# zeahmed/NeuralASR

Hardware: AMD Instinct MI355X
Metric: audio-frames/sec (fwd+bwd+CTC+Adam) at batch 16 per GPU (higher is better)
Workload: dtype f32

## Files before the change

neuralasr_amd/build.py:

```python
import os
import subprocess
import sys
from concurrent.futures import ThreadPoolExecutor

HERE = os.path.dirname(os.path.abspath(__file__))
CSRC = os.path.join(HERE, 'csrc')
LIB = os.path.join(HERE, 'libnasr.so')
KT_LIB = os.path.join(HERE, 'libnasr_kt.so')
KT_SRC = os.path.join(HERE, '..', 'tests', 'kernel_harness', 'harness.hip')
KT_OBJS = ['gemm.o', 'gemm_tph.o', 'optim.o']
SOURCES = ['gemm.hip', 'gemm_tph.hip', 'lstm.hip', 'lstm_persist.hip', 'lstm_wide.hip', 'ctc.hip', 'dense.hip', 'optim.hip', 'nasr_layout.hip',
           'nasr_rec.hip', 'nasr_batch.hip', 'nasr_pass.hip', 'nasr_api.hip', 'nasr_comm.hip', 'beam.cpp',
           'wavenet.hip', 'nasr_wavenet.hip', 'las.hip', 'las_beam.hip', 'nasr_las.hip', 'mfcc.hip', 'resample.hip']
HEADERS = [os.path.join(CSRC, 'kernels.h'), os.path.join(CSRC, 'lstm_device.h'), os.path.join(CSRC, 'nasr_ctx.h'), os.path.join(CSRC, 'wavenet.h'), os.path.join(CSRC, 'las.h'), os.path.join(CSRC, 'las_beam.h'), os.path.join(CSRC, 'resample.h'),
           os.path.join(HERE, '..', 'include', 'nasr.h')]
FLAGS = ['--offload-arch=gfx950', '-O3', '-std=c++17', '-fPIC', '-Wall', '-Wno-unused-function']


def _hipcc():
    for c in (os.environ.get('HIPCC'), '/opt/rocm/bin/hipcc', 'hipcc'):
        if c and (os.path.isabs(c) and os.path.exists(c) or not os.path.isabs(c)):
            return c
    return 'hipcc'


def _stale(target, deps):
    if not os.path.exists(target):
        return True
    t = os.path.getmtime(target)
    return any(os.path.getmtime(d) > t for d in deps if os.path.exists(d))


def build(force=False, verbose=False):
    hipcc = _hipcc()
    bdir = os.path.join(HERE, 'build')
    os.makedirs(bdir, exist_ok=True)
    jobs = []
    objs = []
    for s in SOURCES:
        src = os.path.join(CSRC, s)
        obj = os.path.join(bdir, os.path.splitext(s)[0] + '.o')
        objs.append(obj)
        if force or _stale(obj, [src] + HEADERS):
            jobs.append([hipcc] + FLAGS + ['-c', src, '-o', obj])

    def run(cmd):
        if verbose:
# ... 24 lines not shown
```

neuralasr_amd/csrc/gemm.hip:

```cpp
#include "kernels.h"

namespace nasr {

typedef float f32x16 __attribute__((ext_vector_type(16)));

constexpr int BM = 128, BN = 128, BK = 16, LDT = 132;

struct GemmParams {
  const float* A;
  const float* B;
  float* C;
  int M, N, K, lda, ldb, ldc;
  const int* a_map;
  int a_shift, a_rows;
  const int* c_map;
  const float* bias;
  int split_k, kchunk;
  float* slabs;
};

__device__ __forceinline__ int phys_row(const int* map, int shift, int rows, int logical) {
  int r = map ? map[logical] : logical + shift;
  return (r >= 0 && r < rows) ? r : -1;
}

__device__ __forceinline__ float4 ld4(const float* __restrict__ p) { return *reinterpret_cast<const float4*>(p); }
__device__ __forceinline__ float4 sel4(bool ok, float4 v) {
  return make_float4(ok ? v.x : 0.f, ok ? v.y : 0.f, ok ? v.z : 0.f, ok ? v.w : 0.f);
}

template <bool ACOL, bool BCOL>
__global__ __launch_bounds__(256, 2) void gemm_kernel(GemmParams p) {
  __shared__ __attribute__((aligned(16))) float As[2][BK][LDT];
  __shared__ __attribute__((aligned(16))) float Bs[2][BK][LDT];
  const int tid = threadIdx.x, lane = tid & 63, w = tid >> 6;
  const int m0 = blockIdx.y * BM, n0 = blockIdx.x * BN;
  const int kbeg = blockIdx.z * p.kchunk;
  const int kend = min(p.K, kbeg + p.kchunk);
  const int nk = (kend - kbeg + BK - 1) / BK;
  const float* __restrict__ Ag = p.A;
  const float* __restrict__ Bg = p.B;

  constexpr int NS = BK / 8, KQ = BK / 4;
  bool aok[NS], bok[NS];
  size_t ao[NS], bo[NS];
#pragma unroll
  for (int j = 0; j < NS; ++j) {
    const int idx = tid + 256 * j;
    const int r = idx / KQ, kq = idx % KQ, q = idx & 31;
    if (!ACOL) {
      const int pa = (m0 + r < p.M) ? phys_row(p.a_map, p.a_shift, p.a_rows, m0 + r) : -1;
// ... 78 lines not shown
        nb0 = Bs[buf][k][wn + li]; nb1 = Bs[buf][k][wn + 32 + li];
      }
      acc00 = __builtin_amdgcn_mfma_f32_32x32x2f32(a0, b0, acc00, 0, 0, 0);
      acc01 = __builtin_amdgcn_mfma_f32_32x32x2f32(a0, b1, acc01, 0, 0, 0);
      acc10 = __builtin_amdgcn_mfma_f32_32x32x2f32(a1, b0, acc10, 0, 0, 0);
      acc11 = __builtin_amdgcn_mfma_f32_32x32x2f32(a1, b1, acc11, 0, 0, 0);
      a0 = na0; a1 = na1; b0 = nb0; b1 = nb1;
    }
    if (more) NASR_LSTORE(buf ^ 1);
    __syncthreads();
  }
#undef NASR_GLOAD
#undef NASR_LSTORE

#pragma unroll
  for (int t = 0; t < 4; ++t) {
    const int mi = t >> 1, ni = t & 1;
    const f32x16 acc = t == 0 ? acc00 : t == 1 ? acc01 : t == 2 ? acc10 : acc11;
    const int col = n0 + wn + 32 * ni + li;
    if (col >= p.N) continue;
    const float bv = (p.bias && p.split_k == 1) ? p.bias[col] : 0.f;
#pragma unroll
    for (int r = 0; r < 16; ++r) {
      const int row = m0 + wm + 32 * mi + (r & 3) + 8 * (r >> 2) + 4 * lk;
      if (row >= p.M) continue;
      if (p.split_k > 1) {
        p.slabs[((size_t)blockIdx.z * p.M + row) * p.N + col] = acc[r];
      } else {
        const int pr = p.c_map ? p.c_map[row] : row;
        if (pr >= 0) p.C[(size_t)pr * p.ldc + col] = acc[r] + bv;
      }
    }
  }
}

__global__ __launch_bounds__(256) void gemm_reduce_kernel(GemmParams p) {
  const int64_t n4 = (int64_t)p.M * p.N / 4;
  for (int64_t i = blockIdx.x * (int64_t)blockDim.x + threadIdx.x; i < n4; i += (int64_t)gridDim.x * blockDim.x) {
    const int64_t e = i * 4;
    const int row = (int)(e / p.N), col = (int)(e % p.N);
    float4 s = *reinterpret_cast<const float4*>(p.slabs + e);
    for (int k = 1; k < p.split_k; ++k) {
      const float4 v = *reinterpret_cast<const float4*>(p.slabs + (size_t)k * p.M * p.N + e);
      s.x += v.x; s.y += v.y; s.z += v.z; s.w += v.w;
    }
    if (p.bias) { s.x += p.bias[col]; s.y += p.bias[col + 1]; s.z += p.bias[col + 2]; s.w += p.bias[col + 3]; }
    const int pr = p.c_map ? p.c_map[row] : row;
    if (pr >= 0) *reinterpret_cast<float4*>(p.C + (size_t)pr * p.ldc + col) = s;
  }
}

int gemm_pick_split(int M, int N, int K) {
  const int tiles = ((M + BM - 1) / BM) * ((N + BN - 1) / BN);
  int s = (512 + tiles - 1) / tiles;
  const int max_s = K / 128;
  if (s > max_s) s = max_s;
  if (s < 1) s = 1;
  return s;
}

void launch_gemm(const GemmDesc& g, hipStream_t st) {
  GemmParams p;
  p.A = g.A; p.B = g.B; p.C = g.C;
  p.M = g.M; p.N = g.N; p.K = g.K; p.lda = g.lda; p.ldb = g.ldb; p.ldc = g.ldc;
  p.a_map = g.a_map; p.a_shift = g.a_shift; p.a_rows = g.a_rows; p.c_map = g.c_map; p.bias = g.bias;
  p.split_k = g.split_k < 1 ? 1 : g.split_k;
  p.slabs = g.slabs;
  int kt = (g.K + BK - 1) / BK;
  int per = (kt + p.split_k - 1) / p.split_k;
  p.kchunk = per * BK;
  p.split_k = (kt + per - 1) / per;
  dim3 grid((g.N + BN - 1) / BN, (g.M + BM - 1) / BM, p.split_k), block(256);
  if (!g.a_col && !g.b_col) hipLaunchKernelGGL((gemm_kernel<false, false>), grid, block, 0, st, p);
  else if (g.a_col && !g.b_col) hipLaunchKernelGGL((gemm_kernel<true, false>), grid, block, 0, st, p);
  else if (!g.a_col && g.b_col) hipLaunchKernelGGL((gemm_kernel<false, true>), grid, block, 0, st, p);
  else hipLaunchKernelGGL((gemm_kernel<true, true>), grid, block, 0, st, p);
  if (p.split_k > 1) {
    int64_t n4 = (int64_t)g.M * g.N / 4;
    int blocks = (int)((n4 + 255) / 256);
    if (blocks > 2048) blocks = 2048;
    hipLaunchKernelGGL(gemm_reduce_kernel, dim3(blocks), dim3(256), 0, st, p);
  }
}

}
```

neuralasr_amd/csrc/gemm_tph.hip:

```cpp
#include "kernels.h"

#include <cstdlib>

namespace nasr {

namespace {

typedef _Float16 f16x8 __attribute__((ext_vector_type(8)));
typedef float f32x16 __attribute__((ext_vector_type(16)));
typedef __attribute__((address_space(3))) void* lds_ptr_t;
typedef const __attribute__((address_space(1))) void* gbl_ptr_t;

constexpr int HTB = 1024;
constexpr int TPH_LDS = 2 * 64 * HTB;

__device__ __attribute__((aligned(1024))) unsigned char g_tph_zero[HTB];

__device__ __forceinline__ int tph_slot(int r, int h) { return ((r << 1) | (h ^ ((r >> 3) & 1))) << 4; }

struct GemmTPHParams {
  const unsigned char* A;
  const unsigned char* B;
  float* C;
  int M, N;
  int nkbA, nkbB;
  int kbs;
  int ldc;
  int a_kb_shift;
  const float* bias;
  const float* a_inv;
  const float* b_inv;
  int split_k, kb_chunk;
  float* slabs;
  int nbatch;
  long long a_bstride, b_bstride, c_bstride, ainv_bstride, binv_bstride;
  int a_kb_shift1;
  int swz, gx, gy, gz, pr, pc, pz, sr, sc, sz;
  const int* c_map;
};

__device__ __forceinline__ void emit_h2(const float (&x)[8], float s, unsigned char* dst) {
  f16x8 p1, p2;
#pragma unroll
  for (int e = 0; e < 8; ++e) {
    const float v = x[e] * s;
    const _Float16 h1 = (_Float16)v;
    p1[e] = h1;
    p2[e] = (_Float16)(v - (float)h1);
  }
  *reinterpret_cast<f16x8*>(dst) = p1;
  *reinterpret_cast<f16x8*>(dst + HTB) = p2;
}

}

__global__ __launch_bounds__(256) void absmax_part_kernel(const float* __restrict__ src, int rows, int K, int ld,
                                                          float* __restrict__ rowpart, float* __restrict__ colpart) {
  __shared__ float rm[64][5], cm[4][64];
  const int t = threadIdx.x;
  const int r0 = blockIdx.y * 64, c0 = blockIdx.x * 64;
  const int cq = t & 15, rq = t >> 4;
  float cmax[4] = {0.f, 0.f, 0.f, 0.f};
#pragma unroll
  for (int i = 0; i < 4; ++i) {
    const int r = rq + 16 * i;
    float4 v = make_float4(0.f, 0.f, 0.f, 0.f);
// ... 360 lines not shown
#pragma unroll
        for (int j = 0; j < 2; ++j) acc[i][j] = chain3(acc[i][j], a[i], b[j]);
    }
  }

  const int li = lane & 31, lh = lane >> 5;
  const float* ainv = p.a_inv + (bz ? p.ainv_bstride : 0);
  const float* binv = p.b_inv + (bz ? p.binv_bstride : 0);
#pragma unroll
  for (int mi = 0; mi < TMW; ++mi)
#pragma unroll
    for (int ni = 0; ni < 2; ++ni) {
      const int col = n0 + wn * 64 + 32 * ni + li;
      if (col >= p.N) continue;
      const float bv = (p.bias && p.split_k == 1) ? p.bias[col] : 0.f;
      const float sb = binv[col];
#pragma unroll
      for (int r = 0; r < 16; ++r) {
        const int row = m0 + wm * (32 * TMW) + 32 * mi + (r & 3) + 8 * (r >> 2) + 4 * lh;
        if (row >= p.M) continue;
        const float v = acc[mi][ni][r] * (ainv[row] * sb);
        if (p.split_k > 1) {
          p.slabs[((size_t)bzz * p.M + row) * p.N + col] = v;
        } else {
          if constexpr (CMAP) {
            const int orow = p.c_map[row];
            if (orow >= 0) p.C[(size_t)bz * p.c_bstride + (size_t)orow * p.ldc + col] = v + bv;
          } else {
            p.C[(size_t)bz * p.c_bstride + (size_t)row * p.ldc + col] = v + bv;
          }
        }
      }
    }
}

constexpr int TPH_LDS_SIDE = 2 * 40 * HTB;

hipError_t gemm_tph_prepare() {
  hipError_t e = hipFuncSetAttribute(reinterpret_cast<const void*>(&gemm_tph_kernel<4, 2, 4>),
                                     hipFuncAttributeMaxDynamicSharedMemorySize, TPH_LDS);
  for (const void* f : {reinterpret_cast<const void*>(&gemm_tph_kernel<3, 2, 4>), reinterpret_cast<const void*>(&gemm_tph_kernel<4, 2, 4, true>),
                        reinterpret_cast<const void*>(&gemm_tph_kernel<3, 2, 4, true>)})
    if (e == hipSuccess) e = hipFuncSetAttribute(f, hipFuncAttributeMaxDynamicSharedMemorySize, TPH_LDS);
  if (e == hipSuccess)
    e = hipFuncSetAttribute(reinterpret_cast<const void*>(&gemm_tph_kernel<4, 1, 3>), hipFuncAttributeMaxDynamicSharedMemorySize,
                            TPH_LDS_SIDE);
  return e;
}

int gemm_tph_pick_split(int M, int N, int K, int nbatch) {
  const int tm = gemm_tp_tile_rows(M), tn = 256;
  const int tiles = ((M + tm - 1) / tm) * ((N + tn - 1) / tn) * (nbatch > 1 ? 2 : 1);
  const int kbs = (K + 15) / 16;
  const double kstep = 1.3e-6 * tm / 256.0;
  const double slab = (double)(nbatch > 1 ? 2 : 1) * M * N * 8.0 / 4e12 / kstep;
  int best = 1;
  double best_cost = 1e30;
  for (int s = 1; s <= 64; ++s) {
    if (s > 1 && kbs / s < 32) break;
    const int per = ((kbs + s - 1) / s + 1) & ~1;
    const int rounds = (tiles * s + 255) / 256;
    const double cost = (double)rounds * per + (s > 1 ? s * slab : 0.0);
    if (cost < best_cost - 1e-9) { best_cost = cost; best = s; }
  }
  return best;
}

void launch_gemm_tph(const GemmTPHDesc& g, hipStream_t st) {
  GemmTPHParams p;
  p.A = g.A; p.B = g.B; p.C = g.C; p.M = g.M; p.N = g.N;
  p.nkbA = g.nkbA; p.nkbB = g.nkbB; p.kbs = (g.K + 15) / 16; p.ldc = g.ldc;
  p.a_kb_shift = g.a_kshift / 16;
  p.bias = g.bias; p.a_inv = g.a_inv; p.b_inv = g.b_inv;
  int split = g.split_k < 1 ? 1 : g.split_k;
  const int per = ((p.kbs + split - 1) / split + 1) & ~1;
  p.kb_chunk = per;
  p.split_k = (p.kbs + per - 1) / per;
  p.slabs = g.slabs;
  const int tm = g.side ? 128 : g.tile_rows ? g.tile_rows : gemm_tp_tile_rows(g.M), tn = g.side ? 192 : 256;
  p.nbatch = g.nbatch > 1 ? 2 : 1;
  p.a_bstride = (long long)g.a_bstride; p.b_bstride = (long long)g.b_bstride; p.c_bstride = (long long)g.c_bstride;
  p.ainv_bstride = (long long)g.ainv_bstride; p.binv_bstride = (long long)g.binv_bstride;
  p.a_kb_shift1 = g.a_kshift1 / 16;
  dim3 grid((g.N + tn - 1) / tn, (g.M + tm - 1) / tm, p.split_k * p.nbatch);
  p.c_map = g.c_map;
  p.swz = 0;
  p.gx = (int)grid.x; p.gy = (int)grid.y; p.gz = (int)grid.z;
  p.pr = p.pc = p.pz = 1; p.sr = p.gy; p.sc = p.gx; p.sz = p.gz;
  {
    double best = 1e300;
    const long long total = (long long)p.gx * p.gy * p.gz;
    for (int pz = 1; pz <= 8; pz *= 2)
      for (int pr = 1; pr * pz <= 8; pr *= 2) {
        const int pc = 8 / (pz * pr);
        const int sr = (p.gy + pr - 1) / pr, sc = (p.gx + pc - 1) / pc, sz = (p.gz + pz - 1) / pz;
        const long long padded = 8LL * sr * sc * sz;
        if (padded * 8 > total * 9) continue;
        const double cost = (double)pc * g.M + (double)pr * g.N + 1e-3 * (padded - total);
        if (cost < best) { best = cost; p.swz = 1; p.pr = pr; p.pc = pc; p.pz = pz; p.sr = sr; p.sc = sc; p.sz = sz; }
      }
    if (p.swz) grid = dim3(8 * p.sr * p.sc * p.sz, 1, 1);
  }
  const bool scatter = g.c_map && p.split_k == 1 && !g.side;
  if (g.side) hipLaunchKernelGGL((gemm_tph_kernel<4, 1, 3>), grid, dim3(192), TPH_LDS_SIDE, st, p);
  else if (scatter && tm == 192) hipLaunchKernelGGL((gemm_tph_kernel<3, 2, 4, true>), grid, dim3(512), TPH_LDS, st, p);
  else if (scatter) hipLaunchKernelGGL((gemm_tph_kernel<4, 2, 4, true>), grid, dim3(512), TPH_LDS, st, p);
  else if (tm == 192) hipLaunchKernelGGL((gemm_tph_kernel<3, 2, 4>), grid, dim3(512), TPH_LDS, st, p);
  else hipLaunchKernelGGL((gemm_tph_kernel<4, 2, 4>), grid, dim3(512), TPH_LDS, st, p);
  if (p.split_k > 1) {
    if (g.c_map) launch_reduce_slabs_rows(g.slabs, p.split_k, g.M, g.N, g.ldc, g.c_map, g.C, st);
    else launch_reduce_slabs(g.slabs, p.split_k, (int64_t)p.nbatch * g.M * g.N, g.C, st);
  }
}

}
```

neuralasr_amd/csrc/kernels.h:

```cpp
#pragma once
#include <hip/hip_runtime.h>
#include <stdint.h>

namespace nasr {

const char* test_hook(const char* name);

struct GemmDesc {
  const float* A;
  const float* B;
  float* C;
  int M, N, K;
  int lda, ldb, ldc;
  bool a_col;
  bool b_col;
  const int* a_map;
  int a_shift;
  int a_rows;
  const int* c_map;
  const float* bias;
  int split_k;
  float* slabs;
};
void launch_gemm(const GemmDesc& g, hipStream_t st);
int gemm_pick_split(int M, int N, int K);

int tp_split2_parts(int rows);
int gemm_tp_tile_rows(int M);
size_t tph_bytes(int rows, int K);
size_t tph_scale_ws_floats(int rows, int K);
void launch_tph_scales(const float* src, int rows, int K, int ld, float* row_scale, float* row_inv, float* col_scale,
                       float* col_inv, float* ws, hipStream_t st);
constexpr int TPH_MAX_JOBS = 16;
struct TphScaleJob { const float* src; int rows, K, ld; float *row_scale, *row_inv, *col_scale, *col_inv; };
size_t tph_scale_batch_ws_floats(const TphScaleJob* jobs, int n);
void launch_tph_scales_batch(const TphScaleJob* jobs, int n, float* ws, hipStream_t st);
void launch_tph_scales_from_parts(const float* rowpart, int nrp, int rows, float* row_scale, float* row_inv, const float* colpart,
                                  int ncp, int K, float* col_scale, float* col_inv, hipStream_t st);
void launch_fill(float* p, float v, int n, hipStream_t st);
void launch_tph_split2(const float* src, unsigned char* tpN, unsigned char* tpT, int rows, int K, int ld,
                       const float* row_scale, float rs, const float* col_scale, float cs, float* colpart, hipStream_t st,
                       const int* rowmap = nullptr, const int* rowmap2 = nullptr, int col2 = 0);
void launch_gather_rows(float* dst, const float* src, const int* map, int n, float fill, hipStream_t st);
struct GemmTPHDesc {
  const unsigned char* A;
  const unsigned char* B;
  float* C;
  int M, N, K;
  int nkbA, nkbB;
  int ldc;
  int a_kshift;
  const float* bias;
  const float* a_inv;
  const float* b_inv;
  int split_k;
  float* slabs;
  int tile_rows;
  int nbatch;
  size_t a_bstride, b_bstride;
  int64_t c_bstride, ainv_bstride, binv_bstride;
  int a_kshift1;
  bool side;
  const int* c_map;
};
hipError_t gemm_tph_prepare();
int gemm_tph_pick_split(int M, int N, int K, int nbatch = 1);
void launch_gemm_tph(const GemmTPHDesc& g, hipStream_t st);

struct LstmDims {
  int T, B, Bp, H, Hp, D;
};
void launch_pack_feats(const float* feats_bm, float* X0, int B, int Bp, int T, int F, int Fp, hipStream_t st);
void launch_expand_context(const float* centre, const float* pad, const int* seq_len, float* X0, int B, int Bp, int T,
                           int ctx, int ncep, int Fp, hipStream_t st);
void launch_expand_context_masked(const float* centre, const float* pad, const int* seq_len, const int* masks, int nm,
                                  int static_width, float* X0, int B, int Bp, int T, int ctx, int ncep, int Fp,
                                  hipStream_t st);
void launch_repack_u(const float* U, float* Uf, float* Ub, int Hp, hipStream_t st);
void launch_lstm_fwd_step(const LstmDims& dm, int s, const float* Uf, const float* hin, float* hout, float* gates,
                          float* cbuf, float* out, const int* seq_len, float forget_bias, hipStream_t st);
int lstm_bwd_partials(int Hp);
void launch_lstm_bwd_step(const LstmDims& dm, int s, const float* Ub, const float* pin, float* pout,
                          const float* gates, float* dgbuf, const float* cbuf, const float* dout, const float* dcin,
                          float* dcout, const int* seq_len, hipStream_t st);

struct XcdCtl {
  unsigned xcc_count[8];
  unsigned error;
  unsigned pad[23];
};
static_assert(sizeof(XcdCtl) == 32 * sizeof(unsigned), "the control blocks' head is 32 words");
struct PersistCtl : XcdCtl {
  unsigned flags[8 * 128];
#if defined(NASR_PSTAMP) && NASR_PSTAMP
  unsigned stamps[256][12];
#endif
};
bool persist_supported(int Hp);
size_t persist_image_floats(int Hp, bool bwd);
// ... 81 lines not shown
```

neuralasr_amd/csrc/nasr_ctx.h:

```cpp
#pragma once
#include <hip/hip_runtime.h>

#include <dlfcn.h>
#include <sched.h>
#include <unistd.h>

#include <chrono>

#include <algorithm>
#include <cmath>
#include <cstdio>
#include <cstdlib>
#include <cstring>
#include <functional>
#include <map>
#include <memory>
#include <mutex>
#include <string>
#include <vector>

#include "../../include/nasr.h"
#include "kernels.h"
#include "resample.h"

// ... 240 lines not shown
  static constexpr int NEND = 4;
  StepEnd endw[NEND];
  int end_cur = 0;
  int64_t step_token = 0;
  uint32_t stamp_seq = 0;

  bool resident = false, have_grads = false, have_fwd = false;
  int B = 0, Bp = 0, T = 0, Lmax = 0, Tp = 0, KS = 1;
  int64_t frames = 0;
  std::vector<int32_t> h_seq;
  BatchSlot slots[NSLOT];
  BatchSlot* cur = nullptr;
  Stream cst;
  Stream d2h;
  Event ev_snap;
  DevBuf logits_snap;
  std::mutex slot_mu;
  int slot_rr = 0;
  int32_t *seq_p = nullptr, *lablen_p = nullptr, *labels_p = nullptr, *cstart_p = nullptr, *cpos_p = nullptr,
          *rowmap_p = nullptr;
  bool compactable = false;
  int cmp_rows = 0, cmp_rows_p = 0;
  int32_t *vrow_p = nullptr, *vprev_p = nullptr, *vnext_p = nullptr;
  SV sc_cr, sc_cx;
  DevBuf OTS;

  bool wg_overlap = false;
  bool bwd_lean = false;
  Stream wst;
  Event ev_dx;
  std::vector<Event> ev_wg;
  std::vector<char> wg_pending;
  DevBuf GTTP2, csws2, slabs2;
  SV sc_gc2;
  DevBuf XTP, X0TTP, GTP, GTTP;
  std::vector<DevBuf> OTT;
  std::vector<char> ott_valid;
  DevBuf ctcprobs, ctckexp;
  DevBuf seqbuf, X0, logits, logz, alpha, beta, aoff, boff, logp, nll, loss, slabs, csws, amax, ids, lens,
      stage;
  DevBuf al_logz, al_bp, al_path, al_score, al_logits, al_meta;
  std::vector<DevBuf> gates, outb, cbuf;
  DevBuf dout, hstate, partial, dcstate, dgbuf;

  bool graph_mode = true;
  bool step_decode = false, step_logits = false, have_decoded = false;
  bool step_greedy = false;
  std::map<GraphKey, hipGraphExec_t> graphs;

  bool profiling = false;
  std::vector<Event> ev_pool;
  size_t ev_used = 0;
  struct Span { int ph; hipEvent_t a, b; };
  std::vector<Span> spans;
  Event ev_total_a, ev_total_b;
  bool window_open = false, total_valid = false;
  int n_fwd_launch = 0, n_bwd_launch = 0;
  nasr_phase_times last_times;

  int fail(int code, const std::string& m) {
    t_err = m;
    t_err_handle = this;
    return code;
  }
};

// ... 168 lines not shown
```

neuralasr_amd/csrc/nasr_pass.hip:

```cpp
#include "nasr_ctx.h"

using namespace nasr;
using namespace nasr_impl;

namespace nasr_impl {

int run_steps(nasr_ctx* h, int l, bool bwd, int s0, int s1, hipStream_t st, int* launches) {
  if (h->rec_use != RecKind::Step && s0 == 0 && s1 == h->T) return rec_launch(h, l, bwd, st, launches);
  *launches += s1 - s0;
  const LstmDims dm{h->T, h->B, h->Bp, h->H, h->Hp, h->D};
  const size_t sU = (size_t)l * h->D * h->Hp * h->N4;
  const size_t hs = (size_t)h->D * h->Bp * h->Hp;
  const size_t ps = (size_t)h->D * lstm_bwd_partials(h->Hp) * h->Bp * h->Hp;
  float* hst = h->hstate.as<float>();
  float* par = h->partial.as<float>();
  float* dcs = h->dcstate.as<float>();
  auto body = [&]() {
    if (!bwd) {
      if (s0 == 0) (void)hipMemsetAsync(hst, 0, hs * 4, st);
      for (int s = s0; s < s1; ++s)
        launch_lstm_fwd_step(dm, s, h->Uf + sU, hst + (s & 1) * hs, hst + ((s + 1) & 1) * hs,
                             h->gates[l].as<float>(), h->cbuf[l].as<float>(), h->outb[l].as<float>(),
                             h->seq_p, h->cfg.forget_bias, st);
    } else {
// ... 8 lines not shown
                             dcs + (k & 1) * hs, dcs + ((k + 1) & 1) * hs, h->seq_p, st);
      }
    }
  };
  if (!h->graph_mode) {
    body();
    HIPCHK(h, hipGetLastError());
    return NASR_OK;
  }
  const GraphKey key{h->T, l, bwd ? 1 : 0, s0 * 4096 + (s1 - s0)};
  auto it = h->graphs.find(key);
  if (it == h->graphs.end()) {
    if (h->graphs.size() > 256) drop_graphs(h);
    hipGraph_t g = nullptr;
    HIPCHK(h, hipStreamBeginCapture(st, hipStreamCaptureModeThreadLocal));
    body();
    HIPCHK(h, hipStreamEndCapture(st, &g));
    hipGraphExec_t ex = nullptr;
    HIPCHK(h, hipGraphInstantiate(&ex, g, nullptr, nullptr, 0));
    (void)hipGraphDestroy(g);
    it = h->graphs.emplace(key, ex).first;
  }
  HIPCHK(h, hipGraphLaunch(it->second, st));
  return NASR_OK;
}

float* ensure_slabs(nasr_ctx* h, int split, int M, int N) {
  if (split <= 1) return nullptr;
  bool grew = false;
  if (!h->slabs.ensure((size_t)split * M * N * 4, &grew)) return nullptr;
  return h->slabs.as<float>();
}

int gemm_f32(nasr_ctx* h, GemmDesc g) {
  g.slabs = ensure_slabs(h, g.split_k, g.M, g.N);
  if (g.split_k > 1 && !g.slabs) return h->fail(NASR_ERR_HIP, "slab workspace allocation failed");
  launch_gemm(g, h->st);
  HIPCHK(h, hipGetLastError());
  return NASR_OK;
}

void dg_scales(nasr_ctx* h, int l, int R, bool rows, hipStream_t st) {
  const int DN = h->D * h->N4;
  if (h->dgmax_layer == l) {
    const float* rp = h->dgmax.as<float>();
    launch_tph_scales_from_parts(rp, h->D * 32, R, rows ? h->sc_gr.sp() : nullptr, rows ? h->sc_gr.ip() : nullptr,
                                 rp + (size_t)h->D * 32 * R, 8 / h->D, DN, gc_of(h, l).sp(), gc_of(h, l).ip(), st);
  } else {
    pl_scales(h, dg_of(h, l), R, DN, DN, rows ? &h->sc_gr : nullptr, &gc_of(h, l), st);
  }
}

void gemm_xproj(nasr_ctx* h, int l, int R, hipStream_t st) {
  const int D = h->D, N4 = h->N4, Ip = h->Ip[l];
  const int rows = h->cmp_rows ? h->cmp_rows : R;
  const int* vm = h->cmp_rows ? h->vrow_p : nullptr;
  ActScale as = lstm_in_scale(h, l);
  if (vm && l == 0) { as.rs = h->sc_cx.sp(); as.rinv = h->sc_cx.ip(); }
  const bool both = l > 0 && h->cur && h->cur->has_labels;
  launch_tph_split2(lstm_input(h, l), h->XTP.as<unsigned char>(), both ? h->OTT[l - 1].as<unsigned char>() : nullptr, rows, Ip, Ip,
                    as.rs, 1.f, both ? as.cs : nullptr, 1.f, nullptr, st, vm);
  if (l > 0) h->ott_valid[l - 1] = both;
  GemmTPHDesc g{};
  g.A = h->XTP.as<unsigned char>(); g.B = h->WfTP + h->off_wftp[l]; g.C = h->gates[l].as<float>();
  g.M = rows; g.N = D * N4; g.K = Ip; g.nkbA = (Ip + 15) / 16; g.nkbB = g.nkbA; g.ldc = D * N4;
  g.bias = h->P + h->off_bias[l]; g.split_k = 1;
  g.c_map = vm;
  pl_gemm(g, as.rinv, h->sc_wc[l].ip(), st);
}

void gemm_dx(nasr_ctx* h, int l, int R, hipStream_t st) {
  const int D = h->D, N4 = h->N4;
  const int rows = h->cmp_rows ? h->cmp_rows : R;
  const int* vm = h->cmp_rows ? h->vrow_p : nullptr;
  const float* A = dg_of(h, l);
  float* C = l > 0 ? dout_of(h, l - 1) : h->dYbuf[h->npre - 1].as<float>();
  dg_scales(h, l, R, true, st);
  const float *rs = h->sc_gr.sp(), *rinv = h->sc_gr.ip();
  if (vm) {
    launch_gather_rows(h->sc_cr.sp(), h->sc_gr.sp(), vm, h->cmp_rows_p, 1.f, st);
    launch_gather_rows(h->sc_cr.ip(), h->sc_gr.ip(), vm, h->cmp_rows_p, 1.f, st);
    rs = h->sc_cr.sp(); rinv = h->sc_cr.ip();
  }
  launch_tph_split2(A, h->GTP.as<unsigned char>(), gttp_of(h, l), rows, D * N4, D * N4, rs, 1.f, gc_of(h, l).sp(), 1.f,
                    csws_of(h, l), st, vm);
  h->gttp_layer = l;
  GemmTPHDesc g{};
  g.A = h->GTP.as<unsigned char>(); g.B = h->WbTP + h->off_wbtp[l]; g.C = C;
  g.M = rows; g.N = h->Ip[l]; g.K = D * N4; g.nkbA = (D * N4 + 15) / 16; g.nkbB = g.nkbA; g.ldc = h->Ip[l];
  g.split_k = gemm_tph_pick_split(g.M, g.N, g.K);
  g.slabs = ensure_slabs(h, g.split_k, g.M, g.N);
  if (g.split_k > 1 && !g.slabs) g.split_k = 1;
  g.c_map = vm;
  pl_gemm(g, rinv, h->sc_wr[l].ip(), st);
}

int dense_forward(nasr_ctx* h, int i, const float* X) {
  const int R = h->T * h->Bp, Ip = h->dIp[i], Wp = h->dWp[i];
  const ActScale as = dense_in_scale(h, i);
  pl_split(X, h->XTP.as<unsigned char>(), nullptr, R, Ip, Ip, as.rs, nullptr, nullptr, h->st);
  GemmTPHDesc g{};
  g.A = h->XTP.as<unsigned char>(); g.B = h->DfTP + h->off_dftp[i]; g.C = h->Ybuf[i].as<float>();
  g.M = R; g.N = Wp; g.K = Ip; g.nkbA = (Ip + 15) / 16; g.nkbB = g.nkbA; g.ldc = Wp;
  g.bias = h->P + h->off_db[i]; g.split_k = 1;
  pl_gemm(g, as.rinv, h->sc_dc[i].ip(), h->st);
  launch_dense_act(h->Ybuf[i].as<float>(), R, h->Bp, h->B, h->dWid[i], Wp, h->cfg.relu_clip, h->cfg.dropout[i],
                   h->drop_seed, h->drop_counter, i, h->st);
  pl_scales(h, h->Ybuf[i].as<float>(), R, Wp, Wp, &h->sc_yr[i], &h->sc_yc[i], h->st);
  HIPCHK(h, hipGetLastError());
  return NASR_OK;
}

int dense_backward(nasr_ctx* h, int i, const float* X, float* dX) {
  const int R = h->T * h->Bp, Ip = h->dIp[i], Wp = h->dWp[i];
  const int nkb = (R + 15) / 16;
  float* dZ = h->dYbuf[i].as<float>();
  launch_dense_act_bwd(dZ, h->Ybuf[i].as<float>(), (int64_t)R * Wp, h->cfg.relu_clip, h->cfg.dropout[i], h->st);
  const ActScale as = dense_in_scale(h, i);
  pl_scales(h, dZ, R, Wp, Wp, dX ? &h->sc_gr : nullptr, &h->sc_gc, h->st);
  pl_split(dZ, dX ? h->GTP.as<unsigned char>() : nullptr, h->GTTP.as<unsigned char>(), R, Wp, Wp, h->sc_gr.sp(),
           h->sc_gc.sp(), h->csws.as<float>(), h->st);
  pl_split(X, nullptr, h->DTP.as<unsigned char>(), R, Ip, Ip, nullptr, as.cs, nullptr, h->st);
  {
    GemmTPHDesc g{};
    g.A = h->DTP.as<unsigned char>(); g.B = h->GTTP.as<unsigned char>(); g.C = h->G + h->off_dw[i];
    g.M = Ip; g.N = Wp; g.K = R; g.nkbA = nkb; g.nkbB = nkb; g.ldc = Wp;
    g.split_k = gemm_tph_pick_split(g.M, g.N, g.K);
    g.slabs = ensure_slabs(h, g.split_k, g.M, g.N);
    if (g.split_k > 1 && !g.slabs) return h->fail(NASR_ERR_HIP, "slab workspace allocation failed");
    pl_gemm(g, as.cinv, h->sc_gc.ip(), h->st);
  }
  launch_colsum_parts(h->csws.as<float>(), tp_split2_parts(R), Wp, h->G + h->off_db[i], h->st);
  if (dX) {
    GemmTPHDesc g{};
    g.A = h->GTP.as<unsigned char>(); g.B = h->DbTP + h->off_dbtp[i]; g.C = dX;
    g.M = R; g.N = Ip; g.K = Wp; g.nkbA = (Wp + 15) / 16; g.nkbB = g.nkbA; g.ldc = Ip;
    g.split_k = gemm_tph_pick_split(g.M, g.N, g.K);
    g.slabs = ensure_slabs(h, g.split_k, g.M, g.N);
    if (g.split_k > 1 && !g.slabs) g.split_k = 1;
    pl_gemm(g, h->sc_gr.ip(), h->sc_dr[i].ip(), h->st);
  }
  HIPCHK(h, hipGetLastError());
  return NASR_OK;
}

int forward(nasr_ctx* h) {
  if (!h->resident) return h->fail(NASR_ERR_STATE, "no resident batch: call nasr_upload_batch first");
  switch (h->family) {
    case Family::WaveNet: return wn_forward(h, false);
    case Family::Las: return h->fail(NASR_ERR_STATE, "a LAS handle has no CTC logits: use nasr_las_forward");
    default: break;
  }
  const int Bp = h->Bp, T = h->T, D = h->D, Hp = h->Hp;
  const int R = T * Bp;
  h->n_fwd_launch = 0;
  std::fill(h->ott_valid.begin(), h->ott_valid.end(), 0);
  HIPCHK(h, hipMemsetAsync(h->Gbase, 0, GRAD_HEAD * 4, h->st));
  if (h->rec_use == RecKind::Persist) {
    HIPCHK(h, hipMemsetAsync(h->pctl + 1, 0, (size_t)h->L * sizeof(PersistCtl), h->st));
    HIPCHK(h, hipMemsetAsync(h->xchf, 0, (size_t)h->L * persist_hx_bytes(h->Hp), h->st));
  }
  for (int i = 0; i < h->npre; ++i) {
    PhaseScope ps(h, PH_XPROJ);
    int rc = dense_forward(h, i, i == 0 ? h->X0.as<float>() : h->Ybuf[i - 1].as<float>());
    if (rc) return rc;
  }
  for (int l = 0; l < h->L; ++l) {
    {
      PhaseScope ps(h, PH_XPROJ);
      gemm_xproj(h, l, R, h->st);
      HIPCHK(h, hipGetLastError());
    }
// ... 64 lines not shown
      HIPCHK(h, hipStreamWaitEvent(h->d2h, h->ev_snap, 0));
      HIPCHK(h, hipMemcpyAsync(hp + lg_off, h->logits_snap.p, lg_bytes, hipMemcpyDeviceToHost, h->d2h));
      HIPCHK(h, hipEventRecord(r.ev_lg, h->d2h));
    }
    r.logits = lg_bytes != 0;
    r.seq = ++h->stamp_seq;
    launch_publish_results(h->loss.as<float>(), h->Gbase, h->lens.as<int>(), h->step_greedy ? h->Bp : 0, h->ids.as<int>(),
                           h->step_greedy ? h->B * h->Tp : 0, r.host, r.stamp, r.seq, h->st);
    r.greedy = h->step_greedy;
    r.valid = true; r.B = h->B; r.Bp = h->Bp; r.Tp = h->Tp;
  }
  HIPCHK(h, hipGetLastError());
  return NASR_OK;
}

int loss_pass(nasr_ctx* h, bool training) {
  int rc;
  switch (h->family) {
    case Family::Las: return las_forward(h, true);
    case Family::WaveNet: rc = wn_forward(h, training); break;
    default: rc = forward(h); break;
  }
  return rc ? rc : ctc_forward(h);
}

int weight_grads(nasr_ctx* h, int l, hipStream_t ws, bool side) {
  const int Bp = h->Bp, T = h->T, D = h->D, Hp = h->Hp, N4 = h->N4;
  const int R = T * Bp;
  float* dG = dg_of(h, l);
  unsigned char* GT = gttp_of(h, l);
  float* cs_part = csws_of(h, l);
  nasr_ctx::SV& gc = gc_of(h, l);
  DevBuf& slab_buf = side ? h->slabs2 : h->slabs;
  auto slabs_for = [&](int split, int M, int N) -> float* {
    if (split <= 1) return nullptr;
    bool grew = false;
    return slab_buf.ensure((size_t)split * M * N * 4, &grew) ? slab_buf.as<float>() : nullptr;
  };
  const int rows = h->cmp_rows ? h->cmp_rows : R;
  const int* vm = h->cmp_rows ? h->vrow_p : nullptr;
  const int nkb = (rows + 15) / 16;
  if (h->gttp_layer != l) {
    dg_scales(h, l, R, false, ws);
    launch_tph_split2(dG, nullptr, GT, rows, D * N4, D * N4, nullptr, 1.f, gc.sp(), 1.f, cs_part, ws, vm);
  }
  h->gttp_layer = -1;
  const ActScale ao = act_out(h), ai = lstm_in_scale(h, l);
  for (int m = std::max(l - 1, 0); m <= (vm ? l - 1 : l); ++m)
    if (!h->ott_valid[m]) {
      launch_tph_split2(h->outb[m].as<float>(), nullptr, h->OTT[m].as<unsigned char>(), rows, D * Hp, D * Hp, nullptr, 1.f, ao.cs, 1.f,
                        nullptr, ws, vm);
      h->ott_valid[m] = 1;
    }
  unsigned char* OS = h->OTS.as<unsigned char>() + (wg_alt(h, l) ? tph_bytes(D * Hp, R) : 0);
  if (vm)
    launch_tph_split2(h->outb[l].as<float>(), nullptr, OS, rows, D * Hp, D * Hp, nullptr, 1.f, ao.cs, 1.f, nullptr, ws, h->vprev_p,
                      D == 2 ? h->vnext_p : nullptr, Hp);
  if (l == 0 && h->npre)
    pl_split(lstm_input(h, l), nullptr, h->X0TTP.as<unsigned char>(), R, h->Ip[0], h->Ip[0], nullptr, ai.cs, nullptr, ws);
  {
    GemmTPHDesc g{};
    g.A = l == 0 ? h->X0TTP.as<unsigned char>() : h->OTT[l - 1].as<unsigned char>();
    g.B = GT; g.C = h->G + h->off_wx[l];
    g.M = h->Ip[l]; g.N = D * N4; g.K = rows; g.nkbA = nkb; g.nkbB = nkb; g.ldc = D * N4;
    g.side = side;
    g.split_k = gemm_tph_pick_split(g.M, g.N, g.K);
    g.slabs = slabs_for(g.split_k, g.M, g.N);
    if (g.split_k > 1 && !g.slabs) return h->fail(NASR_ERR_HIP, "slab workspace allocation failed");
    pl_gemm(g, ai.cinv, gc.ip(), ws);
  }
  launch_colsum_parts(cs_part, tp_split2_parts(rows), D * N4, h->G + h->off_bias[l], ws);
  {
    GemmTPHDesc g{};
    g.A = vm ? OS : h->OTT[l].as<unsigned char>(); g.B = GT; g.C = h->G + h->off_u[(size_t)l * D];
    g.M = Hp; g.N = N4; g.K = rows; g.nkbA = nkb; g.nkbB = nkb; g.ldc = N4;
    g.a_kshift = vm ? 0 : -Bp;
    g.nbatch = D;
    g.a_bstride = (size_t)(Hp / 32) * pl_rb_bytes(nkb); g.b_bstride = (size_t)(N4 / 32) * pl_rb_bytes(nkb);
    g.c_bstride = (int64_t)Hp * N4;
    g.a_kshift1 = vm ? 0 : Bp;
    g.side = side;
    g.split_k = gemm_tph_pick_split(g.M, g.N, g.K, D);
    g.slabs = slabs_for(g.split_k * D, g.M, g.N);
    if (g.split_k > 1 && !g.slabs) return h->fail(NASR_ERR_HIP, "slab workspace allocation failed");
    pl_gemm(g, ao.cinv, gc.ip(), ws, Hp, N4);
  }
  HIPCHK(h, hipGetLastError());
  return NASR_OK;
}

int wg_join(nasr_ctx* h, int l) {
  if (l >= 0 && l < h->L && h->wg_pending[l]) {
    HIPCHK(h, hipStreamWaitEvent(h->st, h->ev_wg[l], 0));
    h->wg_pending[l] = 0;
  }
  return NASR_OK;
}

int backward(nasr_ctx* h) {
  switch (h->family) {
    case Family::WaveNet: return wn_backward(h);
    case Family::Las: return las_backward(h);
    default: break;
  }
  const int Bp = h->Bp, T = h->T, D = h->D, Hp = h->Hp;
  const int R = T * Bp, Rp = h->Tp * Bp;
  const bool sr = h->cfg.merge == NASR_MERGE_STACK_RESHAPE && D == 2;
  if (h->rec_use == RecKind::Persist) {
    HIPCHK(h, hipMemsetAsync(h->pctl + 1 + h->L, 0, (size_t)h->L * sizeof(PersistCtl), h->st));
    HIPCHK(h, hipMemsetAsync(h->xchb, 0, (size_t)h->L * persist_px_bytes(), h->st));
  }
  {
    PhaseScope ps(h, PH_PROJCTC);
    const CtcDims d = ctc_dims(h);
    launch_ctc_grad(d, h->logits.as<float>(), h->logz.as<float>(), h->lablen_p, h->seq_p,
                    h->cstart_p, h->cpos_p, h->alpha.as<float>(), h->beta.as<float>(),
                    h->aoff.as<double>(), h->boff.as<double>(), h->logp.as<double>(), 1.f / (float)h->B, h->st);
// ... 88 lines not shown
```

Baseline: 1.227 million.

## Fuse split-K reduction into GEMM via last-arriving-block ticket counters

Removes the separate split-K reduce kernels after the f32 and TPH GEMMs. Each output tile's K-slices now increment an atomic ticket counter, and the last slice to arrive sums all slabs and writes C, with bias and row mapping. This saves a kernel launch and lets the reduction overlap with other tiles still computing. In exchange it adds atomics, fences and per-context ticket buffers, and falls back to no split when a module ticket array would overflow.

```diff
diff --git a/neuralasr_amd/build.py b/neuralasr_amd/build.py
--- a/neuralasr_amd/build.py
+++ b/neuralasr_amd/build.py
@@ -12,7 +12,7 @@
 SOURCES = ['gemm.hip', 'gemm_tph.hip', 'lstm.hip', 'lstm_persist.hip', 'lstm_wide.hip', 'ctc.hip', 'dense.hip', 'optim.hip', 'nasr_layout.hip',
            'nasr_rec.hip', 'nasr_batch.hip', 'nasr_pass.hip', 'nasr_api.hip', 'nasr_comm.hip', 'beam.cpp',
            'wavenet.hip', 'nasr_wavenet.hip', 'las.hip', 'las_beam.hip', 'nasr_las.hip', 'mfcc.hip', 'resample.hip']
-HEADERS = [os.path.join(CSRC, 'kernels.h'), os.path.join(CSRC, 'lstm_device.h'), os.path.join(CSRC, 'nasr_ctx.h'), os.path.join(CSRC, 'wavenet.h'), os.path.join(CSRC, 'las.h'), os.path.join(CSRC, 'las_beam.h'), os.path.join(CSRC, 'resample.h'),
+HEADERS = [os.path.join(CSRC, 'kernels.h'), os.path.join(CSRC, 'lstm_device.h'), os.path.join(CSRC, 'nasr_ctx.h'), os.path.join(CSRC, 'wavenet.h'), os.path.join(CSRC, 'las.h'), os.path.join(CSRC, 'las_beam.h'), os.path.join(CSRC, 'resample.h'), os.path.join(CSRC, 'splitk_ticket.h'),
            os.path.join(HERE, '..', 'include', 'nasr.h')]
 FLAGS = ['--offload-arch=gfx950', '-O3', '-std=c++17', '-fPIC', '-Wall', '-Wno-unused-function']
 
diff --git a/neuralasr_amd/csrc/gemm.hip b/neuralasr_amd/csrc/gemm.hip
--- a/neuralasr_amd/csrc/gemm.hip
+++ b/neuralasr_amd/csrc/gemm.hip
@@ -1,4 +1,5 @@
 #include "kernels.h"
+#include "splitk_ticket.h"
 
 namespace nasr {
 
@@ -17,6 +18,7 @@
   const float* bias;
   int split_k, kchunk;
   float* slabs;
+  unsigned* tickets;
 };
 
 __device__ __forceinline__ int phys_row(const int* map, int shift, int rows, int logical) {
@@ -161,21 +163,43 @@
       }
     }
   }
-}
-
-__global__ __launch_bounds__(256) void gemm_reduce_kernel(GemmParams p) {
-  const int64_t n4 = (int64_t)p.M * p.N / 4;
-  for (int64_t i = blockIdx.x * (int64_t)blockDim.x + threadIdx.x; i < n4; i += (int64_t)gridDim.x * blockDim.x) {
-    const int64_t e = i * 4;
-    const int row = (int)(e / p.N), col = (int)(e % p.N);
-    float4 s = *reinterpret_cast<const float4*>(p.slabs + e);
+  if (p.split_k == 1) return;
+
+  unsigned* ticket = (p.tickets ? p.tickets : g_splitk_tickets) + (size_t)blockIdx.y * gridDim.x + blockIdx.x;
+  if (!splitk_arrive_last(ticket, p.split_k, reinterpret_cast<unsigned*>(&As[0][0][0]))) return;
+  constexpr int C4 = BN / 4, ITER = BM * C4 / 256, UNR = 4;
+  const size_t sstride = (size_t)p.M * p.N;
+  for (int i0 = 0; i0 < ITER; i0 += UNR) {
+    float4 s[UNR];
+    size_t off[UNR];
+    int orow[UNR], ocol[UNR];
+#pragma unroll
+    for (int u = 0; u < UNR; ++u) {
+      const int idx = tid + 256 * (i0 + u);
+      const int row = m0 + idx / C4, col = n0 + 4 * (idx % C4);
+      const bool ok = row < p.M && col < p.N;
+      orow[u] = !ok ? -1 : p.c_map ? p.c_map[row] : row;
+      ocol[u] = col;
+      off[u] = (size_t)row * p.N + col;
+      s[u] = orow[u] >= 0 ? *reinterpret_cast<const float4*>(p.slabs + off[u]) : make_float4(0.f, 0.f, 0.f, 0.f);
+    }
     for (int k = 1; k < p.split_k; ++k) {
-      const float4 v = *reinterpret_cast<const float4*>(p.slabs + (size_t)k * p.M * p.N + e);
-      s.x += v.x; s.y += v.y; s.z += v.z; s.w += v.w;
-    }
-    if (p.bias) { s.x += p.bias[col]; s.y += p.bias[col + 1]; s.z += p.bias[col + 2]; s.w += p.bias[col + 3]; }
-    const int pr = p.c_map ? p.c_map[row] : row;
-    if (pr >= 0) *reinterpret_cast<float4*>(p.C + (size_t)pr * p.ldc + col) = s;
+#pragma unroll
+      for (int u = 0; u < UNR; ++u) {
+        if (orow[u] < 0) continue;
+        const float4 v = *reinterpret_cast<const float4*>(p.slabs + (size_t)k * sstride + off[u]);
+        s[u].x += v.x; s[u].y += v.y; s[u].z += v.z; s[u].w += v.w;
+      }
+    }
+#pragma unroll
+    for (int u = 0; u < UNR; ++u) {
+      if (orow[u] < 0) continue;
+      if (p.bias) {
+        const int col = ocol[u];
+        s[u].x += p.bias[col]; s[u].y += p.bias[col + 1]; s[u].z += p.bias[col + 2]; s[u].w += p.bias[col + 3];
+      }
+      *reinterpret_cast<float4*>(p.C + (size_t)orow[u] * p.ldc + ocol[u]) = s[u];
+    }
   }
 }
 
@@ -188,28 +212,37 @@
   return s;
 }
 
+namespace {
+void gemm_slices(const GemmDesc& g, int* kchunk, int* split) {
+  int s = g.split_k < 1 ? 1 : g.split_k;
+  const long long tiles = (long long)((g.N + BN - 1) / BN) * ((g.M + BM - 1) / BM);
+  if (!g.tickets && tiles > SPLITK_MODULE_TICKETS) s = 1;
+  const int kt = (g.K + BK - 1) / BK;
+  const int per = (kt + s - 1) / s;
+  *kchunk = per * BK;
+  *split = per > 0 ? (kt + per - 1) / per : 1;
+}
+}
+
+int gemm_tickets(const GemmDesc& g) {
+  int kchunk, split;
+  gemm_slices(g, &kchunk, &split);
+  return split > 1 ? ((g.N + BN - 1) / BN) * ((g.M + BM - 1) / BM) : 0;
+}
+
 void launch_gemm(const GemmDesc& g, hipStream_t st) {
   GemmParams p;
   p.A = g.A; p.B = g.B; p.C = g.C;
   p.M = g.M; p.N = g.N; p.K = g.K; p.lda = g.lda; p.ldb = g.ldb; p.ldc = g.ldc;
   p.a_map = g.a_map; p.a_shift = g.a_shift; p.a_rows = g.a_rows; p.c_map = g.c_map; p.bias = g.bias;
-  p.split_k = g.split_k < 1 ? 1 : g.split_k;
   p.slabs = g.slabs;
-  int kt = (g.K + BK - 1) / BK;
-  int per = (kt + p.split_k - 1) / p.split_k;
-  p.kchunk = per * BK;
-  p.split_k = (kt + per - 1) / per;
+  p.tickets = g.tickets;
+  gemm_slices(g, &p.kchunk, &p.split_k);
   dim3 grid((g.N + BN - 1) / BN, (g.M + BM - 1) / BM, p.split_k), block(256);
   if (!g.a_col && !g.b_col) hipLaunchKernelGGL((gemm_kernel<false, false>), grid, block, 0, st, p);
   else if (g.a_col && !g.b_col) hipLaunchKernelGGL((gemm_kernel<true, false>), grid, block, 0, st, p);
   else if (!g.a_col && g.b_col) hipLaunchKernelGGL((gemm_kernel<false, true>), grid, block, 0, st, p);
   else hipLaunchKernelGGL((gemm_kernel<true, true>), grid, block, 0, st, p);
-  if (p.split_k > 1) {
-    int64_t n4 = (int64_t)g.M * g.N / 4;
-    int blocks = (int)((n4 + 255) / 256);
-    if (blocks > 2048) blocks = 2048;
-    hipLaunchKernelGGL(gemm_reduce_kernel, dim3(blocks), dim3(256), 0, st, p);
-  }
-}
-
-}
+}
+
+}
diff --git a/neuralasr_amd/csrc/gemm_tph.hip b/neuralasr_amd/csrc/gemm_tph.hip
--- a/neuralasr_amd/csrc/gemm_tph.hip
+++ b/neuralasr_amd/csrc/gemm_tph.hip
@@ -1,4 +1,5 @@
 #include "kernels.h"
+#include "splitk_ticket.h"
 
 #include <cstdlib>
 
@@ -32,6 +33,7 @@
   const float* b_inv;
   int split_k, kb_chunk;
   float* slabs;
+  unsigned* tickets;
   int nbatch;
   long long a_bstride, b_bstride, c_bstride, ainv_bstride, binv_bstride;
   int a_kb_shift1;
@@ -458,6 +460,41 @@
         }
       }
     }
+  if (p.split_k == 1) return;
+
+  unsigned* ticket = (p.tickets ? p.tickets : g_splitk_tickets) + ((size_t)bz * p.gy + by) * p.gx + bx;
+  if (!splitk_arrive_last(ticket, p.split_k, reinterpret_cast<unsigned*>(lds))) return;
+  constexpr int C4 = TN / 4, NTH = 64 * NWV, ITER = TM * C4 / NTH, UNR = 4;
+  static_assert(TM * C4 % (NTH * UNR) == 0, "reducer: the tile is a whole number of passes");
+  const size_t sstride = (size_t)p.nbatch * p.M * p.N;
+  const float* slab0 = p.slabs + (size_t)bz * p.M * p.N;
+  float* Cb = p.C + (size_t)bz * p.c_bstride;
+  for (int i0 = 0; i0 < ITER; i0 += UNR) {
+    float4 s[UNR];
+    size_t off[UNR];
+    int orow[UNR], ocol[UNR];
+#pragma unroll
+    for (int u = 0; u < UNR; ++u) {
+      const int idx = tid + NTH * (i0 + u);
+      const int row = m0 + idx / C4, col = n0 + 4 * (idx % C4);
+      const bool ok = row < p.M && col < p.N;
+      orow[u] = !ok ? -1 : p.c_map ? p.c_map[row] : row;
+      ocol[u] = col;
+      off[u] = (size_t)row * p.N + col;
+      s[u] = orow[u] >= 0 ? *reinterpret_cast<const float4*>(slab0 + off[u]) : make_float4(0.f, 0.f, 0.f, 0.f);
+    }
+    for (int k = 1; k < p.split_k; ++k) {
+#pragma unroll
+      for (int u = 0; u < UNR; ++u) {
+        if (orow[u] < 0) continue;
+        const float4 v = *reinterpret_cast<const float4*>(slab0 + (size_t)k * sstride + off[u]);
+        s[u].x += v.x; s[u].y += v.y; s[u].z += v.z; s[u].w += v.w;
+      }
+    }
+#pragma unroll
+    for (int u = 0; u < UNR; ++u)
+      if (orow[u] >= 0) *reinterpret_cast<float4*>(Cb + (size_t)orow[u] * p.ldc + ocol[u]) = s[u];
+  }
 }
 
 constexpr int TPH_LDS_SIDE = 2 * 40 * HTB;
@@ -492,23 +529,45 @@
   return best;
 }
 
+namespace {
+struct TphGrid { int tm, tn, gx, gy, nbatch, kb_chunk, split; };
+TphGrid tph_grid(const GemmTPHDesc& g) {
+  TphGrid t;
+  t.tm = g.side ? 128 : g.tile_rows ? g.tile_rows : gemm_tp_tile_rows(g.M);
+  t.tn = g.side ? 192 : 256;
+  t.gx = (g.N + t.tn - 1) / t.tn; t.gy = (g.M + t.tm - 1) / t.tm;
+  t.nbatch = g.nbatch > 1 ? 2 : 1;
+  const int kbs = (g.K + 15) / 16;
+  int split = g.split_k < 1 ? 1 : g.split_k;
+  if (!g.tickets && (long long)t.gx * t.gy * t.nbatch > SPLITK_MODULE_TICKETS) split = 1;
+  t.kb_chunk = ((kbs + split - 1) / split + 1) & ~1;
+  t.split = (kbs + t.kb_chunk - 1) / t.kb_chunk;
+  return t;
+}
+}
+
+int gemm_tph_tickets(const GemmTPHDesc& g) {
+  const TphGrid t = tph_grid(g);
+  return t.split > 1 ? t.gx * t.gy * t.nbatch : 0;
+}
+
 void launch_gemm_tph(const GemmTPHDesc& g, hipStream_t st) {
   GemmTPHParams p;
   p.A = g.A; p.B = g.B; p.C = g.C; p.M = g.M; p.N = g.N;
   p.nkbA = g.nkbA; p.nkbB = g.nkbB; p.kbs = (g.K + 15) / 16; p.ldc = g.ldc;
   p.a_kb_shift = g.a_kshift / 16;
   p.bias = g.bias; p.a_inv = g.a_inv; p.b_inv = g.b_inv;
-  int split = g.split_k < 1 ? 1 : g.split_k;
-  const int per = ((p.kbs + split - 1) / split + 1) & ~1;
-  p.kb_chunk = per;
-  p.split_k = (p.kbs + per - 1) / per;
+  const TphGrid t = tph_grid(g);
+  p.kb_chunk = t.kb_chunk;
+  p.split_k = t.split;
   p.slabs = g.slabs;
-  const int tm = g.side ? 128 : g.tile_rows ? g.tile_rows : gemm_tp_tile_rows(g.M), tn = g.side ? 192 : 256;
-  p.nbatch = g.nbatch > 1 ? 2 : 1;
+  p.tickets = g.tickets;
+  const int tm = t.tm;
+  p.nbatch = t.nbatch;
   p.a_bstride = (long long)g.a_bstride; p.b_bstride = (long long)g.b_bstride; p.c_bstride = (long long)g.c_bstride;
   p.ainv_bstride = (long long)g.ainv_bstride; p.binv_bstride = (long long)g.binv_bstride;
   p.a_kb_shift1 = g.a_kshift1 / 16;
-  dim3 grid((g.N + tn - 1) / tn, (g.M + tm - 1) / tm, p.split_k * p.nbatch);
+  dim3 grid(t.gx, t.gy, p.split_k * p.nbatch);
   p.c_map = g.c_map;
   p.swz = 0;
   p.gx = (int)grid.x; p.gy = (int)grid.y; p.gz = (int)grid.z;
@@ -533,10 +592,6 @@
   else if (scatter) hipLaunchKernelGGL((gemm_tph_kernel<4, 2, 4, true>), grid, dim3(512), TPH_LDS, st, p);
   else if (tm == 192) hipLaunchKernelGGL((gemm_tph_kernel<3, 2, 4>), grid, dim3(512), TPH_LDS, st, p);
   else hipLaunchKernelGGL((gemm_tph_kernel<4, 2, 4>), grid, dim3(512), TPH_LDS, st, p);
-  if (p.split_k > 1) {
-    if (g.c_map) launch_reduce_slabs_rows(g.slabs, p.split_k, g.M, g.N, g.ldc, g.c_map, g.C, st);
-    else launch_reduce_slabs(g.slabs, p.split_k, (int64_t)p.nbatch * g.M * g.N, g.C, st);
-  }
-}
-
-}
+}
+
+}
diff --git a/neuralasr_amd/csrc/kernels.h b/neuralasr_amd/csrc/kernels.h
--- a/neuralasr_amd/csrc/kernels.h
+++ b/neuralasr_amd/csrc/kernels.h
@@ -21,9 +21,11 @@
   const float* bias;
   int split_k;
   float* slabs;
+  unsigned* tickets;
 };
 void launch_gemm(const GemmDesc& g, hipStream_t st);
 int gemm_pick_split(int M, int N, int K);
+int gemm_tickets(const GemmDesc& g);
 
 int tp_split2_parts(int rows);
 int gemm_tp_tile_rows(int M);
@@ -62,9 +64,11 @@
   int a_kshift1;
   bool side;
   const int* c_map;
+  unsigned* tickets;
 };
 hipError_t gemm_tph_prepare();
 int gemm_tph_pick_split(int M, int N, int K, int nbatch = 1);
+int gemm_tph_tickets(const GemmTPHDesc& g);
 void launch_gemm_tph(const GemmTPHDesc& g, hipStream_t st);
 
 struct LstmDims {
diff --git a/neuralasr_amd/csrc/nasr_ctx.h b/neuralasr_amd/csrc/nasr_ctx.h
--- a/neuralasr_amd/csrc/nasr_ctx.h
+++ b/neuralasr_amd/csrc/nasr_ctx.h
@@ -296,6 +296,7 @@
   std::vector<Event> ev_wg;
   std::vector<char> wg_pending;
   DevBuf GTTP2, csws2, slabs2;
+  DevBuf tickets, tickets2;
   SV sc_gc2;
   DevBuf XTP, X0TTP, GTP, GTTP;
   std::vector<DevBuf> OTT;
diff --git a/neuralasr_amd/csrc/nasr_pass.hip b/neuralasr_amd/csrc/nasr_pass.hip
--- a/neuralasr_amd/csrc/nasr_pass.hip
+++ b/neuralasr_amd/csrc/nasr_pass.hip
@@ -64,9 +64,26 @@
   return h->slabs.as<float>();
 }
 
+unsigned* ensure_tickets(DevBuf& buf, int n, hipStream_t st) {
+  if (n <= 0) return nullptr;
+  bool grew = false;
+  if (!buf.ensure((size_t)std::max(n, 4096) * sizeof(unsigned), &grew)) return nullptr;
+  if (grew && hipMemsetAsync(buf.p, 0, buf.cap, st) != hipSuccess) return nullptr;
+  return buf.as<unsigned>();
+}
+bool splitk_ws(nasr_ctx* h, GemmTPHDesc& g, hipStream_t st) {
+  g.slabs = ensure_slabs(h, g.split_k * (g.nbatch > 1 ? 2 : 1), g.M, g.N);
+  g.tickets = g.slabs ? ensure_tickets(h->tickets, gemm_tph_tickets(g), st) : nullptr;
+  return g.split_k <= 1 || (g.slabs && (g.tickets || !gemm_tph_tickets(g)));
+}
+
 int gemm_f32(nasr_ctx* h, GemmDesc g) {
   g.slabs = ensure_slabs(h, g.split_k, g.M, g.N);
   if (g.split_k > 1 && !g.slabs) return h->fail(NASR_ERR_HIP, "slab workspace allocation failed");
+  if (const int nt = gemm_tickets(g)) {
+    g.tickets = ensure_tickets(h->tickets, nt, h->st);
+    if (!g.tickets) return h->fail(NASR_ERR_HIP, "split-K counter allocation failed");
+  }
   launch_gemm(g, h->st);
   HIPCHK(h, hipGetLastError());
   return NASR_OK;
@@ -121,8 +138,7 @@
   g.A = h->GTP.as<unsigned char>(); g.B = h->WbTP + h->off_wbtp[l]; g.C = C;
   g.M = rows; g.N = h->Ip[l]; g.K = D * N4; g.nkbA = (D * N4 + 15) / 16; g.nkbB = g.nkbA; g.ldc = h->Ip[l];
   g.split_k = gemm_tph_pick_split(g.M, g.N, g.K);
-  g.slabs = ensure_slabs(h, g.split_k, g.M, g.N);
-  if (g.split_k > 1 && !g.slabs) g.split_k = 1;
+  if (!splitk_ws(h, g, st)) g.split_k = 1;
   g.c_map = vm;
   pl_gemm(g, rinv, h->sc_wr[l].ip(), st);
 }
@@ -158,8 +174,7 @@
     g.A = h->DTP.as<unsigned char>(); g.B = h->GTTP.as<unsigned char>(); g.C = h->G + h->off_dw[i];
     g.M = Ip; g.N = Wp; g.K = R; g.nkbA = nkb; g.nkbB = nkb; g.ldc = Wp;
     g.split_k = gemm_tph_pick_split(g.M, g.N, g.K);
-    g.slabs = ensure_slabs(h, g.split_k, g.M, g.N);
-    if (g.split_k > 1 && !g.slabs) return h->fail(NASR_ERR_HIP, "slab workspace allocation failed");
+    if (!splitk_ws(h, g, h->st)) return h->fail(NASR_ERR_HIP, "slab workspace allocation failed");
     pl_gemm(g, as.cinv, h->sc_gc.ip(), h->st);
   }
   launch_colsum_parts(h->csws.as<float>(), tp_split2_parts(R), Wp, h->G + h->off_db[i], h->st);
@@ -168,8 +183,7 @@
     g.A = h->GTP.as<unsigned char>(); g.B = h->DbTP + h->off_dbtp[i]; g.C = dX;
     g.M = R; g.N = Ip; g.K = Wp; g.nkbA = (Wp + 15) / 16; g.nkbB = g.nkbA; g.ldc = Ip;
     g.split_k = gemm_tph_pick_split(g.M, g.N, g.K);
-    g.slabs = ensure_slabs(h, g.split_k, g.M, g.N);
-    if (g.split_k > 1 && !g.slabs) g.split_k = 1;
+    if (!splitk_ws(h, g, h->st)) g.split_k = 1;
     pl_gemm(g, h->sc_gr.ip(), h->sc_dr[i].ip(), h->st);
   }
   HIPCHK(h, hipGetLastError());
@@ -300,10 +314,15 @@
   float* cs_part = csws_of(h, l);
   nasr_ctx::SV& gc = gc_of(h, l);
   DevBuf& slab_buf = side ? h->slabs2 : h->slabs;
-  auto slabs_for = [&](int split, int M, int N) -> float* {
-    if (split <= 1) return nullptr;
+  DevBuf& ticket_buf = side ? h->tickets2 : h->tickets;
+  auto ws_for = [&](GemmTPHDesc& g) -> bool {
+    if (g.split_k <= 1) return true;
     bool grew = false;
-    return slab_buf.ensure((size_t)split * M * N * 4, &grew) ? slab_buf.as<float>() : nullptr;
+    if (!slab_buf.ensure((size_t)g.split_k * (g.nbatch > 1 ? 2 : 1) * g.M * g.N * 4, &grew)) return false;
+    g.slabs = slab_buf.as<float>();
+    const int nt = gemm_tph_tickets(g);
+    g.tickets = ensure_tickets(ticket_buf, nt, ws);
+    return g.tickets || !nt;
   };
   const int rows = h->cmp_rows ? h->cmp_rows : R;
   const int* vm = h->cmp_rows ? h->vrow_p : nullptr;
@@ -333,8 +352,7 @@
     g.M = h->Ip[l]; g.N = D * N4; g.K = rows; g.nkbA = nkb; g.nkbB = nkb; g.ldc = D * N4;
     g.side = side;
     g.split_k = gemm_tph_pick_split(g.M, g.N, g.K);
-    g.slabs = slabs_for(g.split_k, g.M, g.N);
-    if (g.split_k > 1 && !g.slabs) return h->fail(NASR_ERR_HIP, "slab workspace allocation failed");
+    if (!ws_for(g)) return h->fail(NASR_ERR_HIP, "slab workspace allocation failed");
     pl_gemm(g, ai.cinv, gc.ip(), ws);
   }
   launch_colsum_parts(cs_part, tp_split2_parts(rows), D * N4, h->G + h->off_bias[l], ws);
@@ -349,8 +367,7 @@
     g.a_kshift1 = vm ? 0 : Bp;
     g.side = side;
     g.split_k = gemm_tph_pick_split(g.M, g.N, g.K, D);
-    g.slabs = slabs_for(g.split_k * D, g.M, g.N);
-    if (g.split_k > 1 && !g.slabs) return h->fail(NASR_ERR_HIP, "slab workspace allocation failed");
+    if (!ws_for(g)) return h->fail(NASR_ERR_HIP, "slab workspace allocation failed");
     pl_gemm(g, ao.cinv, gc.ip(), ws, Hp, N4);
   }
   HIPCHK(h, hipGetLastError());
diff --git a/neuralasr_amd/csrc/splitk_ticket.h b/neuralasr_amd/csrc/splitk_ticket.h
--- /dev/null
+++ b/neuralasr_amd/csrc/splitk_ticket.h
@@ -0,0 +1,30 @@
+#pragma once
+#include <hip/hip_runtime.h>
+
+namespace nasr {
+
+constexpr int SPLITK_MODULE_TICKETS = 4096;
+namespace {
+__device__ unsigned g_splitk_tickets[SPLITK_MODULE_TICKETS];
+}
+
+__device__ __forceinline__ bool splitk_arrive_last(unsigned* ticket, int split, unsigned* lds_word) {
+  asm volatile("s_waitcnt vmcnt(0)" ::: "memory");
+  __syncthreads();
+  if (threadIdx.x == 0) {
+    __builtin_amdgcn_fence(__ATOMIC_RELEASE, "agent");
+    asm volatile("s_waitcnt vmcnt(0)" ::: "memory");
+    const unsigned t = __hip_atomic_fetch_add(ticket, 1u, __ATOMIC_RELAXED, __HIP_MEMORY_SCOPE_AGENT);
+    const bool last = t == (unsigned)(split - 1);
+    if (last) {
+      __hip_atomic_store(ticket, 0u, __ATOMIC_RELAXED, __HIP_MEMORY_SCOPE_AGENT);
+      __builtin_amdgcn_fence(__ATOMIC_ACQUIRE, "agent");
+      asm volatile("s_waitcnt vmcnt(0)" ::: "memory");
+    }
+    *lds_word = last ? 1u : 0u;
+  }
+  __syncthreads();
+  return *lds_word != 0u;
+}
+
+}
```

Measured after the change: 1.094 million. 0.892x the previous value.
